# Genomics-HSE/MiSTI

Measured on AMD Instinct MI355X. Metric: composite-llk evals/sec over (split×mi) grid, 128 merged PSMC intervals, higher is better.
Workload: dtype f64; 1 GPU; config2: numT=128, 64x64 split x mi-rate grid, one band, --cpfit; candidates_per_gpu=4096, candidates_total=4096, replicates=1, numT=128, batches_in_flight=20, streams=20, world_size=1, parallelism=1 GPU

## Files before the change

misti_amd/csrc/misti_api.cpp:

```cpp
#include <cassert>
#include <hip/hip_runtime.h>

#include <cmath>
#include <chrono>
#include <complex>
#include <thread>
#include <cstdarg>
#include <cstdio>
#include <cstring>
#include <mutex>
#include <string>
#include <vector>

#include "misti_device.h"
#include "misti_tables.hpp"

namespace {

thread_local std::string g_err;

int fail(int code, const char* fmt, ...) {
    char buf[512];
    va_list ap;
    va_start(ap, fmt);
// ... 37 lines not shown
        size_t want = bytes + bytes / 4 + 4096;
        hipError_t e = hipHostMalloc(&p, want, hipHostMallocDefault);
        if (e == hipSuccess) cap = want;
        return e;
    }
    void release() { if (p) (void)hipHostFree(p); p = nullptr; cap = 0; }
};
constexpr size_t PIN_STAGE_MAX = (size_t)256 << 20;

}

struct misti_ctx {
    int device = 0;
    misti::DevModel dm{};
    int unfolded = 0;
    hipStream_t own_stream = nullptr;
    hipStream_t stream = nullptr;
    DevBuf model_f64, model_i32;
    DevBuf consts;
    DevBuf scan_v, scan_i;
    DevBuf prof_v, prof_i, prof_idx;
    DevBuf ws_jafs, ws_status;
    DevBuf ws_order;
    DevBuf ws_diag;
    int64_t diag_n = 0;
    int32_t* hint_host = nullptr;
    int32_t* hint_dev = nullptr;
    int32_t batch_seq = 0;
    misti::Tuning tune;
    int table_cur = 0;
    size_t table_clean[2] = {0, 0};
    DevBuf ws_trunk;
    DevBuf ws_chain_f64, ws_chain_i32;
    DevBuf st_split, st_params, st_bounds, st_pulses, st_jsfs, st_llk, st_jafs, st_lc, st_pr, st_status;
    PinBuf pin_in, pin_out;
    std::vector<char> heap_in, heap_out;
    bool trace = false;
    DevBuf ws_solver, ws_iters;
    DevBuf ws_post;
    int64_t trace_n = 0, trace_iter_cap = 0;
    const int32_t* trace_of = nullptr;
    hipEvent_t order_ev = nullptr;
    hipEvent_t last_ev = nullptr;
    bool last_ev_set = false;
    unsigned hints = 0;
    hipStream_t side_stream = nullptr;
// ... 149 lines not shown
    if (n_cand == 0) return 0;
    if (!d_split) return fail(MISTI_E_ARG, "split_time is NULL");
    if (c->hints & MISTI_HINT_INTEGER_SPLITS) hints |= RUN_INTEGER_SPLITS;
    if (c->dm.n_param > 0 && !d_params) return fail(MISTI_E_ARG, "params is NULL but the model has %d parameters", c->dm.n_param);
    if (n_rep > 0 && (!d_jsfs || !d_llk)) return fail(MISTI_E_ARG, "jsfs / llk is NULL with n_rep > 0");
    HIP_TRY(hipSetDevice(c->device));
    if (!d_jafs) { HIP_TRY(c->ws_jafs.reserve((size_t)n_cand * 7 * sizeof(double))); d_jafs = c->ws_jafs.as<double>(); }
    if (!d_status) { HIP_TRY(c->ws_status.reserve((size_t)n_cand * sizeof(int32_t))); d_status = c->ws_status.as<int32_t>(); }
    if (n_cand > INT32_MAX / 8) return fail(MISTI_E_LIMIT, "n_cand too large for one call");
    const size_t nc = (size_t)n_cand, numT = (size_t)c->dm.numT;
    const size_t tsize = misti::chain_table_size(n_cand);
    const int64_t follow_max_h = c->tune.follow_max > 0 ? c->tune.follow_max : misti::FOLLOW_MAX_CHAINS;
    const size_t ntr = ((hints & RUN_UNSHARED) && n_cand > follow_max_h) ? 0 : (size_t)misti::trunk_capacity(n_cand, c->tune);
    const size_t f64_n = nc * numT * 2 + nc * (numT + 1) * 6 + nc * 6 + nc * 2 + nc * 6;
    const size_t set_n = 4 + 4 * tsize;
    const size_t i32_n = 2 * set_n + 10 * nc + ntr;
    HIP_TRY(c->ws_chain_f64.reserve(f64_n * sizeof(double)));
    {
        void* before = c->ws_chain_i32.p;
        HIP_TRY(c->ws_chain_i32.reserve(i32_n * sizeof(int32_t)));
        if (c->ws_chain_i32.p != before) c->table_clean[0] = c->table_clean[1] = 0;
    }
    HIP_TRY(c->ws_order.reserve(nc * sizeof(int32_t)));
    if (ntr) HIP_TRY(c->ws_trunk.reserve(ntr * numT * misti::TRUNK_REC * sizeof(double)));
    if (n_rep > 0) HIP_TRY(c->consts.reserve((size_t)n_rep * sizeof(double)));
    misti::ChainBufs cb;
    {
        double* d = c->ws_chain_f64.as<double>();
        cb.lc = d; d += nc * numT * 2;
        cb.trace = d; d += nc * (numT + 1) * 6;
        cb.work = d; d += nc * 6;
        cb.tail_lc = d; d += nc * 2;
        cb.tail_state = d;
        int32_t* q = c->ws_chain_i32.as<int32_t>();
        const int cur = c->table_cur;
        int32_t* set[2] = {q, q + set_n};
        q += 2 * set_n;
        if (c->table_clean[cur] != tsize) HIP_TRY(hipMemsetAsync(set[cur], 0, set_n * sizeof(int32_t), c->stream));
        c->table_clean[cur] = 0;
        c->table_clean[cur ^ 1] = 0;
        cb.n_chains = set[cur]; cb.table = set[cur] + 4; cb.slot_chain = cb.table + tsize; cb.slot_len = cb.slot_chain + tsize;
        cb.slot_keep = cb.slot_len + tsize;
        cb.z_n_chains = set[cur ^ 1]; cb.z_table = set[cur ^ 1] + 4; cb.z_slot_len = cb.z_table + 2 * tsize; cb.z_slot_keep = cb.z_slot_len + tsize;
        cb.slot_of = q; q += nc; cb.of = q; q += nc; cb.chain_slot = q; q += nc; cb.rep = q; q += nc;
        cb.fail_t = q; q += nc; cb.fail_status = q; q += nc; cb.tail_status = q; q += nc; cb.chain_order = q; q += nc; cb.resume_t = q; q += nc; cb.resume_list = q; q += nc;
        cb.trunk_ok = q;
        cb.tmask = (uint32_t)(tsize - 1);
        cb.trunk = ntr ? c->ws_trunk.as<double>() : nullptr;
        cb.trunk_cap = (int64_t)ntr;
        cb.hint = c->hint_dev;
        cb.simd_load = c->tune.pairing ? pair_table(c->device) : nullptr;
        cb.bounds = c->dm.n_band > 0 ? d_bounds : nullptr;
        cb.pulse_times = c->dm.n_pulse > 0 ? d_pulses : nullptr;
        cb.integer_splits = (hints & RUN_INTEGER_SPLITS) ? 1 : 0;
        cb.post_lam = nullptr;
        cb.post_word = nullptr;
        if (!(c->dm.flags & MISTI_CPFIT)) {
            HIP_TRY(c->ws_post.reserve(nc * (numT + 1) * (sizeof(double) + sizeof(int32_t))));
            cb.post_lam = c->ws_post.as<double>();
            if (c->trace) cb.post_word = reinterpret_cast<int32_t*>(cb.post_lam + nc * (numT + 1));
        }
        cb.solver = cb.tail_solver = cb.cand_solver = nullptr;
        cb.iters = nullptr;
        cb.iter_cap = 0;
        c->trace_n = 0;
        c->trace_iter_cap = 0;
        if (c->trace) {
            HIP_TRY(c->ws_solver.reserve((nc * numT + nc + nc * (numT + 1)) * sizeof(int32_t)));
            HIP_TRY(hipMemsetAsync(c->ws_solver.p, 0, (nc * numT + nc + nc * (numT + 1)) * sizeof(int32_t), c->stream));
// ... 280 lines not shown
    if (hipEventCreateWithFlags(&c->last_ev, hipEventDisableTiming) != hipSuccess) { (void)hipGetLastError(); c->last_ev = nullptr; }
    {
        std::lock_guard<std::mutex> lock(g_ctx_mu);
        g_ctxs.push_back(c);
    }
    guard.keep = true;
    *out = c;
    return 0;
}

int misti_create(const misti_model_t* model, int device, misti_ctx** out) { return misti_create_prio_(model, device, 0, out); }

int misti_destroy(misti_ctx* c) {
    if (!c) return 0;
    {
        std::lock_guard<std::mutex> lock(g_ctx_mu);
        for (size_t i = 0; i < g_ctxs.size(); ++i) if (g_ctxs[i] == c) { g_ctxs.erase(g_ctxs.begin() + (long)i); break; }
    }
    (void)hipSetDevice(c->device);
    if (c->stream) (void)hipStreamSynchronize(c->stream);
    if (c->own_stream && c->own_stream != c->stream) (void)hipStreamSynchronize(c->own_stream);
    if (c->side_stream) (void)hipStreamSynchronize(c->side_stream);
    (void)hipGetLastError();
    for (auto* b : {&c->model_f64, &c->model_i32, &c->consts, &c->ws_jafs, &c->ws_status, &c->ws_chain_f64, &c->ws_chain_i32, &c->ws_order, &c->ws_diag, &c->ws_trunk, &c->ws_solver, &c->ws_iters, &c->ws_post,
                    &c->st_split, &c->st_params, &c->st_bounds, &c->st_pulses, &c->st_jsfs, &c->st_llk, &c->st_jafs, &c->st_lc, &c->st_pr, &c->st_status, &c->nm_f64, &c->nm_i32, &c->scan_v, &c->scan_i, &c->prof_v, &c->prof_i, &c->prof_idx, &c->curv_f64, &c->curv_i32, &c->boot_chunks, &c->param_totals})
        b->release();
    c->pin_in.release();
    c->pin_out.release();
    if (c->nm_live_host) (void)hipHostFree(c->nm_live_host);
    if (c->hint_host) (void)hipHostFree(c->hint_host);
    for (int w = 0; w < 3; ++w)
        for (auto& pr : c->pending[w]) { (void)hipEventDestroy(pr.first); (void)hipEventDestroy(pr.second); }
    for (hipEvent_t e : {c->order_ev, c->last_ev, c->packed_ev, c->side_ev}) if (e) (void)hipEventDestroy(e);
    if (c->side_stream) (void)hipStreamDestroy(c->side_stream);
    if (c->own_stream) (void)hipStreamDestroy(c->own_stream);
    (void)hipGetLastError();
    delete c;
    return 0;
}

int misti_set_stream(misti_ctx* c, void* s) {
    if (!c) return fail(MISTI_E_ARG, "ctx is NULL");
    hipStream_t next = s ? static_cast<hipStream_t>(s) : c->own_stream;
    if (next == c->stream) return 0;
    HIP_TRY(hipSetDevice(c->device));
    if (!c->order_ev) HIP_TRY(hipEventCreateWithFlags(&c->order_ev, hipEventDisableTiming));
    HIP_TRY(hipEventRecord(c->order_ev, c->stream));
// ... 1046 lines not shown
```

misti_amd/csrc/misti_device.h:

```cpp
#pragma once
#include <hip/hip_runtime.h>
#include <stdint.h>

#include "../../include/misti_hip.h"

#include "misti_consts.h"

namespace misti {

struct DevTables {
    int src[MAXNZ][64];
    int kind[MAXNZ][64];
    int mult[MAXNZ][64];
    int dcnt[4][64];
    int jaf[7][64];
    int jaf1[7][NS1];
    unsigned long long jaf_bits[7][3];
    unsigned int jaf1_bits[7];
    int grp_lo[NS1], grp_hi[NS1];
    int anc_n[2], anc_dst[2], anc_src[2][8];
    int pulse_n[2][64];
    int pulse_src[2][64][MAXPULSE];
    int pulse_ab[2][64][MAXPULSE];
    double tal_zr[TALBOT_HALF], tal_zi[TALBOT_HALF];
    double tal_cr[TALBOT_HALF], tal_ci[TALBOT_HALF];
};

struct DevModel {
    int numT;
    int sample_date;
    unsigned flags;
    int n_band, n_pulse, n_param;
    double mixture_th;
    const double* times;
    const double* lh;
    const int* run_start;
    const int* run_end;
    const int* leave_ok;
    misti_band_t bands[MISTI_MAX_BANDS];
    misti_pulse_t pulses[MISTI_MAX_PULSES];
};

struct ChainBufs {
    int32_t* n_chains;
    int32_t* z_n_chains;
    int32_t* z_table;
    int32_t* z_slot_len;
    int32_t* z_slot_keep;
    int32_t* table;
    int32_t* slot_chain;
    int32_t* slot_len;
    int32_t* slot_keep;
    int32_t* resume_t;
    int32_t* resume_list;
    int32_t* chain_order;
    int32_t* slot_of;
    int32_t* of;
    int32_t* chain_slot;
    int32_t* rep;
    uint32_t tmask;
    double* lc;
    double* trace;
    int32_t* fail_t;
    int32_t* fail_status;
    double* work;
    double* tail_lc;
    double* tail_state;
    int32_t* tail_status;
    double* trunk;
    int32_t* trunk_ok;
    int64_t trunk_cap;
    int32_t* simd_load;
    int32_t* hint;
    int32_t seq;
    int32_t unsorted;
    int32_t integer_splits;
    const int32_t* bounds;
    const int32_t* pulse_times;
    double* post_lam;
    int32_t* post_word;
    int32_t* solver;
    int32_t* tail_solver;
    int32_t* cand_solver;
    double* iters;
    int64_t iter_cap;
};

__host__ __device__ __forceinline__ int32_t solver_word(int nfev, int status, int kind) {
    return (int32_t)((nfev & 0xffff) | ((status & 15) << 16) | ((kind & 15) << 20));
}

__device__ __forceinline__ int64_t chain_of(const ChainBufs& cb, int64_t cand) { return cb.of[cand]; }
__device__ __forceinline__ int chain_len(const ChainBufs& cb, int64_t ch) { return cb.slot_len[cb.chain_slot[ch]]; }

enum { NM_NONE = 0, NM_REFLECT = 1, NM_EXPAND = 2, NM_CONTRACT = 3, NM_INSIDE = 4,
       NM_CUT = 5 };
struct NmBatch {
    double* pts;
    double* split;
    int32_t* row;
    int32_t* bnd;
    int32_t* put;
    double* par;
};
enum { NM_B_INIT, NM_B_REFLECT, NM_B_SECOND, NM_B_SHRINK, NM_B_SPEC, NM_BATCHES };
struct NmState {
    int64_t S;
    int N;
    int maxiter;
    int64_t maxfun;
    double xatol, fatol;
    double split;
    const double* split_of;
    const int32_t* row_of;
    const int32_t* bounds_of;
// ... 120 lines not shown
```

misti_amd/csrc/misti_kernels.hip:

```cpp
#include <hip/hip_runtime.h>
#include <math.h>
#include <stdint.h>
#include <stdlib.h>

#include "misti_device.h"
#include "misti_score.h"

namespace misti {

__constant__ DevTables c_tab;
__constant__ double c_inv[INV_TABLE];
constexpr int QMAX_TABLE = 320;
__constant__ double c_qmax[QMAX_TABLE];

constexpr double Q_SWITCH = 96.0;
constexpr int JACOBI_MAX = 600;
constexpr int JACOBI_WATCH = 32;
constexpr int JACOBI_FLOOR = 48;
constexpr double JACOBI_BLOWUP = 1e12;
constexpr int SUBSTEP_MAX = 256;
constexpr long long FOLLOW_SPIN_LIMIT = 1LL << 22;

__device__ __forceinline__ int lane_id() { return threadIdx.x & 63; }

// ... 1686 lines not shown
#endif
#ifdef MISTI_STAMP
            r[0] = (double)c_tree; r[1] = (double)(c_collect + c_update); r[2] = (double)c_next;
            r[3] = (double)c_adv; r[4] = (double)c_batch; r[5] = (double)c_book;
#endif
        } else {
            cb.tail_status[cand] = status;
        }
    }
}

#ifndef MISTI_DEFAULT_FIT_WAVES
#define MISTI_DEFAULT_FIT_WAVES 1
#endif
#ifndef MISTI_FOLLOW_WAVES
#define MISTI_FOLLOW_WAVES 2
#endif
template <bool CPFIT, int GROUP>
__global__ __launch_bounds__(64) __attribute__((amdgpu_waves_per_eu(CPFIT ? 2 : MISTI_DEFAULT_FIT_WAVES, CPFIT ? 2 : MISTI_DEFAULT_FIT_WAVES)))
void correct_kernel(DevModel m, int64_t n_items, ChainBufs cb, const double* __restrict__ split_time, const double* __restrict__ params, int yield_nfev) {
    extern __shared__ double lds[];
    {
        const int64_t i = (int64_t)blockIdx.x * 64 + threadIdx.x;
        if (i < n_items) cb.of[i] = cb.slot_chain[cb.slot_of[i]];
    }
    correct_body<CPFIT, GROUP, false>(m, n_items, cb, split_time, params, (int64_t)blockIdx.x, lds, nullptr, nullptr, nullptr, cb.chain_order,
                                      GROUP == 64 ? 0 : yield_nfev);
}

template <bool CPFIT>
__global__ __launch_bounds__(64) __attribute__((amdgpu_waves_per_eu(CPFIT ? MISTI_FOLLOW_WAVES : 1, CPFIT ? MISTI_FOLLOW_WAVES : 1)))
void correct_resume_kernel(DevModel m, int64_t n_items, ChainBufs cb, const double* __restrict__ split_time, const double* __restrict__ params) {
    extern __shared__ double lds[];
    __shared__ int next;
    const int n_res = cb.n_chains[3];
    if ((int)blockIdx.x >= n_res) return;
    __builtin_amdgcn_s_setprio(3);
    double* pre = lds + 3 * (size_t)m.numT;
    for (;;) {
        if (threadIdx.x == 0) next = atomicAdd(&cb.n_chains[2], 1);
        __syncthreads();
        const int pos = next;
        __syncthreads();
        if (pos >= n_res) break;
        const int64_t ch = cb.resume_list[pos];
        correct_body<CPFIT, 64, false, true>(m, n_items, cb, split_time, params, ch, lds, nullptr, nullptr, pre, nullptr, 0, cb.resume_t[ch]);
        __syncthreads();
// ... 146 lines not shown
            const double gr = T * zr * zz, gi = -T * zi * zz;
            accp += 2.0 * wr;
            acci += 2.0 * (wr * gr - wi * gi);
        }
        if (solved) {
            x = accp; wint = acci;
        } else {
            const int n_sub = (int)ceil(q / Q_SWITCH);
            if (n_sub > SUBSTEP_MAX) return MISTI_STIFF;
            const double2 r = series_substeps(R.srcl[0], R.srcl[1], R.srcl[2], R.srcl[3], cf[0], cf[1], cf[2], cf[3], xbuf, lane, n_sub, q, T, dT, x);
            x = r.x; wint = r.y;
        }
    }
    if (t < m.sample_date) w_pre += wint; else w_post += wint;
    return MISTI_OK;
}

__device__ __forceinline__ double run_mean(const double* lc, int k, int a, int b, const Grid& G) {
    double acc = 0.0, tt = 0.0;
    for (int j = a; j < b; ++j) { double Tj = G.T(j); acc += lc[2 * j + k] * Tj; tt += Tj; }
    return acc / tt;
}

__device__ __forceinline__ void smooth_rates(const DevModel& m, const Grid& G, double* lcb, int lane, int lo, int bound) {
    double sm[SMOOTH_REPS][2];
#pragma unroll
    for (int rep = 0; rep < SMOOTH_REPS; ++rep) {
        sm[rep][0] = sm[rep][1] = 0.0;
        if (rep * 64 >= bound || rep * 64 + 63 < lo) continue;
        int t = rep * 64 + lane;
        for (int k = 0; k < 2; ++k) {
            double v = 0.0;
            if (t >= lo && t < bound) {
                int a = m.run_start[k * m.numT + t];
                int b = m.run_end[k * m.numT + t];
                if (b > bound) b = bound;
                v = run_mean(lcb, k, a, b, G);
            }
            sm[rep][k] = v;
        }
    }
    lds_fence();
#pragma unroll
    for (int rep = 0; rep < SMOOTH_REPS; ++rep) {
        int t = rep * 64 + lane;
        if (t >= lo && t < bound) { lcb[2 * t] = sm[rep][0]; lcb[2 * t + 1] = sm[rep][1]; }
    }
    lds_fence();
}

__device__ __forceinline__ bool trunk_active(const ChainBufs& cb, int64_t n_cand) {
    const int64_t nch = cb.n_chains[0];
    return cb.trunk_cap > 0 && nch <= cb.trunk_cap && nch * TRUNK_MIN_SHARE <= n_cand;
}

__device__ __forceinline__
void trunk_body(const DevModel& m, int64_t n_cand, const double* __restrict__ params, const ChainBufs& cb, int64_t ch, double* lds, int phase = 0) {
    const int lane = lane_id();
    if (!trunk_active(cb, n_cand) || ch >= cb.n_chains[0]) return;
    if (wrong_phase(cb, ch, phase)) return;
    double* xbuf = lds;
    double* lcb = lds + 128;
    const int ft = cb.fail_t[ch];
    int Lt = chain_len(cb, ch);
    if (ft < Lt) Lt = ft;
    const double* par = params ? params + (int64_t)cb.rep[ch] * m.n_param : nullptr;
    Grid G;
    G.times = m.times; G.lh = m.lh; G.numT0 = m.numT; G.numT = m.numT; G.split = Lt; G.ins = -1; G.frac = 0.0;
    Model mod{&m, par, Lt, {0, 0, 0, 0}};
    mod.bb = cb.bounds ? cb.bounds + (int64_t)cb.rep[ch] * 2 * m.n_band : nullptr;
    mod.pt = cb.pulse_times ? cb.pulse_times + (int64_t)cb.rep[ch] * m.n_pulse : nullptr;
// ... 80 lines not shown
        const int cut = have >= need ? len : have;
        if (t >= cut) break;
        if (b0 > cut) b0 = cut;
        if (b1 > cut) b1 = cut;
        const double l0 = smooth ? run_mean(lc_sh, 0, a0, b0, G) : lc_sh[2 * t];
        const double l1 = smooth ? run_mean(lc_sh, 1, a1, b1, G) : lc_sh[2 * t + 1];
        if (lane == 0) { lcb[2 * t] = l0; lcb[2 * t + 1] = l1; }
        lds_fence();
        if (t == m.sample_date) ancient_project(xbuf, lane, x);
        if (twopop_interval(R, m, mod, G, lcb, xbuf, lane, t, x, w_pre, w_post) != MISTI_OK) break;
    }
    if (!stored) store(ok, xs, ws0, ws1);
    if (lane == 0) cb.trunk_ok[ch] = ok;
}

template <bool CPFIT>
__global__ __launch_bounds__(128) __attribute__((amdgpu_waves_per_eu(CPFIT ? MISTI_FOLLOW_WAVES : 1, CPFIT ? MISTI_FOLLOW_WAVES : 1)))
void correct_follow_kernel(DevModel m, int64_t n_items, ChainBufs cb, const double* __restrict__ split_time, const double* __restrict__ params) {
    extern __shared__ double lds[];
    double* tk = lds + 3 * (size_t)m.numT;
    double* lc_sh = tk + 128 + 2 * (size_t)(m.numT + 1);
    volatile int* flags = (volatile int*)(lc_sh + 2 * (size_t)m.numT);
    double* pre = lc_sh + 2 * (size_t)m.numT + 4;
    for (int64_t i = (int64_t)blockIdx.x * 128 + threadIdx.x; i < n_items; i += (int64_t)gridDim.x * 128) cb.of[i] = cb.slot_chain[cb.slot_of[i]];
    const int64_t n_live = cb.n_chains[0];
    if ((int64_t)blockIdx.x >= n_live) return;
    int* next = (int*)(flags + 2);
    bool chain_role = threadIdx.x < 64;
    int32_t* my_load = nullptr;
    if (cb.simd_load) {
        int* ex = next + 1;
        const unsigned hw = __builtin_amdgcn_s_getreg((31 << 11) | 4);
        const unsigned xcc = __builtin_amdgcn_s_getreg((3 << 11) | 20);
        const int simd = (hw >> 4) & 3;
        if ((threadIdx.x & 63) == 0) ex[threadIdx.x >> 6] = simd;
        if (threadIdx.x == 0) ex[2] = (int)((((xcc & 7) * 8 + ((hw >> 13) & 7)) * 2 + ((hw >> 12) & 1)) * 16 + ((hw >> 8) & 15)) * 4;
        __syncthreads();
        if (threadIdx.x == 0) {
            int32_t* t = cb.simd_load + ex[2];
            const int c0 = __hip_atomic_load(&t[ex[0]], __ATOMIC_RELAXED, __HIP_MEMORY_SCOPE_AGENT);
            const int c1 = __hip_atomic_load(&t[ex[1]], __ATOMIC_RELAXED, __HIP_MEMORY_SCOPE_AGENT);
            const int sw = c1 < c0 ? 1 : 0;
            ex[3] = sw;
            atomicAdd(&t[ex[sw]], 1);
        }
        __syncthreads();
        chain_role = ((int)(threadIdx.x >> 6) ^ ex[3]) == 0;
// ... 56 lines not shown
    const double lh0 = G.lhk(t, 0), lh1 = G.lhk(t, 1);
    const double pa = exp(nc0), pb = exp(nc1);
    const double w0 = pa / (pa + pb), w1 = pb / (pa + pb);
    const double Te = w0 * ect_one_pop(lh0, T) + w1 * ect_one_pop(lh1, T);
    double x[1] = {w0 * lh0 + w1 * lh1};
    auto resid = [&](const double l[1], double f[1]) { f[0] = ect_one_pop(l[0], T) - Te; };
    const int32_t word = trf_bounded<1>(resid, x, 0.01 * fmin(lh0, lh1));
    cb.post_lam[gid] = x[0];
    if (cb.post_word) cb.post_word[gid] = word;
}

template <bool CPFIT, int WPB = WAVES_PER_BLOCK>
__global__ __launch_bounds__(WPB * 64, 4)
void spectrum_kernel(DevModel m, int64_t n_cand, const int32_t* __restrict__ order, const double* __restrict__ split_time, const double* __restrict__ params,
                     ChainBufs cb, double* __restrict__ lc_out, double* __restrict__ pr_out,
                     double* __restrict__ jafs_out, int32_t* __restrict__ status_out, double* __restrict__ diag_out,
                     int n_inline, const double* __restrict__ jsfs, const double* __restrict__ consts, double* __restrict__ llk_out, int phase) {
    extern __shared__ double lds[];
    const int lane = lane_id();
    const int wave = __builtin_amdgcn_readfirstlane((int)(threadIdx.x >> 6));
    const int64_t slot = (int64_t)blockIdx.x * WPB + wave;
    if (slot >= n_cand) return;
    if (phase != 0) {
        const int64_t cd = (int64_t)__builtin_amdgcn_readfirstlane(order[slot]);
        if (wrong_phase(cb, (int64_t)__builtin_amdgcn_readfirstlane((int)chain_of(cb, cd)), phase)) return;
    }
#ifdef MISTI_STAMP2
    long long s_[8];
#define KSTAMP(i) s_[i] = clock64();
#else
#define KSTAMP(i)
#endif
    KSTAMP(0)
    const int64_t cand = (int64_t)__builtin_amdgcn_readfirstlane(order[slot]);
    const int lc_rows = m.numT + 1;
    double* xbuf = lds + (size_t)wave * (128 + 2 * lc_rows);
    double* lcb = xbuf + 128;
    const double* par = params ? params + cand * m.n_param : nullptr;
    Grid G;
    const int32_t* bb = cb.bounds ? cb.bounds + cand * 2 * m.n_band : nullptr;
    const int32_t* pt = cb.pulse_times ? cb.pulse_times + cand * m.n_pulse : nullptr;
    int status = setup_candidate(m, split_time[cand], par, G, bb, pt);
    if (status == MISTI_OK && cb.integer_splits && G.ins >= 0) status = MISTI_BAD_STRUCTURE;
    Model mod{&m, par, G.split, {0, 0, 0, 0}};
    mod.bb = bb;
    mod.pt = pt;
    mod.cache();
    const int64_t ch = (int64_t)__builtin_amdgcn_readfirstlane((int)chain_of(cb, cand));
    const int nfull = (G.ins >= 0) ? G.ins : G.split;
    const double* lc_ch = cb.lc + ch * (int64_t)m.numT * 2;
    const double* tr_ch = cb.trace + ch * (int64_t)(m.numT + 1) * 6;
    int have = 0;
    if (status == MISTI_OK) {
        const int ft = cb.fail_t[ch];
        if (ft < nfull) { status = cb.fail_status[ch]; have = ft + 1; }
        else {
            have = nfull;
            if (G.ins >= 0) { const int ts = cb.tail_status[cand]; have = nfull + 1; if (ts != MISTI_OK) status = ts; }
        }
    }
    double* lc_o = lc_out ? lc_out + cand * (int64_t)lc_rows * 2 : nullptr;
    double* pr_o = pr_out ? pr_out + cand * (int64_t)(m.numT + 2) * 6 : nullptr;
    int32_t* sv_o = cb.cand_solver ? cb.cand_solver + cand * (int64_t)lc_rows : nullptr;
    if (sv_o) {
        for (int i = lane; i < lc_rows; i += 64) {
            int32_t wd = 0;
            if (i < nfull && i < have) wd = cb.solver[ch * (int64_t)m.numT + i];
            else if (i == nfull && G.ins >= 0 && have > nfull) wd = cb.tail_solver[cand];
            sv_o[i] = wd;
        }
    }
    if (pr_o) {
        const int rows = (status == MISTI_OK) ? G.split + 1 : (have > nfull ? nfull + 1 : (have > 0 ? have : (status == MISTI_OK ? 1 : 0)));
        for (int i = lane; i < (m.numT + 2) * 6; i += 64) {
            const int r = i / 6, j = i - 6 * r;
            double v = 0.0;
            if (r == m.numT + 1) v = cb.work[ch * 6 + j];
            else if (r < rows) v = (G.ins >= 0 && r == nfull + 1) ? cb.tail_state[cand * 6 + j] : tr_ch[6 * r + j];
            pr_o[i] = v;
        }
    }
    if (status != MISTI_OK) {
        if (lane == 0) { status_out[cand] = status; if (diag_out) diag_out[cand] = NAN; }
        if (lane < 7) jafs_out[cand * 7 + lane] = NAN;
        if (lane < n_inline) llk_out[cand * n_inline + lane] = -INFINITY;
        if (lc_o)
            for (int i = lane; i < 2 * lc_rows; i += 64) {
                const int t = i >> 1;
                lc_o[i] = (t < have && t < nfull) ? lc_ch[i] : (t < have && t == nfull && G.ins >= 0) ? cb.tail_lc[2 * cand + (i & 1)] : 0.0;
            }
        return;
    }
    KSTAMP(1)
    for (int i = lane; i < 2 * lc_rows; i += 64) {
        const int t = i >> 1;
        lcb[i] = (t < nfull) ? lc_ch[i] : (t == nfull && G.ins >= 0) ? cb.tail_lc[2 * cand + (i & 1)] : 0.0;
    }
    lds_fence();
    {
        double mx = 0.0;
        for (int t = lane; t < G.split; t += 64) { double T = G.T(t); mx = fmax(mx, fmax(lcb[2 * t], lcb[2 * t + 1]) * T); }
        for (int o = 32; o > 0; o >>= 1) mx = fmax(mx, __shfl_xor(mx, o, 64));
        if (diag_out && lane == 0) diag_out[cand] = (m.flags & MISTI_TRUE_EPS) ? 0.0 : mx;
    }
    int t0 = 0;
    const bool use_trunk = trunk_active(cb, n_cand);
    int smooth_from = 0;
    if (use_trunk) {
        const int t_own = trunk_leave(m, G);
        t0 = min(t_own, cb.trunk_ok[ch]);
        if (t0 == t_own && !lc_o) smooth_from = t_own;
    }
    KSTAMP(2)
    {
        const double* stt = (G.ins >= 0) ? cb.tail_state + 6 * cand : tr_ch + 6 * nfull;
        const double nc0 = (stt[0] + stt[2]) + stt[4], nc1 = (stt[1] + stt[3]) + stt[5];
        const double delta = nc1 - nc0;
        const double ed = exp(delta);
        const int last = G.numT - 1;
        for (int base = G.split; base < G.numT; base += 64) {
            int t = base + lane;
            if (t < last) {
                double T = G.T(t);
                double lam = 1.0;
                int32_t word = 0;
                if (T != 0) {
                    double lh0 = G.lhk(t, 0), lh1 = G.lhk(t, 1);
                    if (CPFIT) {
                        double pnc = (exp(-T * lh0) + exp(delta - T * lh1)) / (1.0 + ed);
                        lam = -log(pnc) / T;
                        word = solver_word(0, 0, 1);
                    } else {
                        lam = cb.post_lam[cand * lc_rows + t];
                        word = cb.post_word ? cb.post_word[cand * lc_rows + t] : 0;
                    }
                }
                lcb[2 * t] = lam; lcb[2 * t + 1] = lam;
                if (sv_o) sv_o[t] = word;
            } else if (t == last) {
                double lh0 = G.lhk(t, 0), lh1 = G.lhk(t, 1);
                double lam = (1.0 + ed) / (1.0 / lh0 + ed / lh1);
                lcb[2 * t] = lam; lcb[2 * t + 1] = lam;
                if (sv_o) sv_o[t] = solver_word(0, 0, 1);
            }
        }
        lds_fence();
        KSTAMP(3)
        if (m.flags & MISTI_SMOOTH) smooth_rates(m, G, lcb, lane, smooth_from, G.split);
        for (int i = lane; i < 2 * G.numT; i += 64) { double v = lcb[i]; if (!(v == v)) status = MISTI_NUMERIC; }
        status = __any(status != MISTI_OK) ? MISTI_NUMERIC : MISTI_OK;
        if (lc_o) for (int i = lane; i < 2 * lc_rows; i += 64) lc_o[i] = (i < 2 * G.numT) ? lcb[i] : 0.0;
    }
    double jn = NAN;
    KSTAMP(4)
    KSTAMP(5) KSTAMP(6) KSTAMP(7)

    if (status == MISTI_OK) {
        TwoPopRow R;
        R.load(lane);
        const bool live = R.live;
        double x = (lane == 2) ? 1.0 : 0.0;
        double w_pre = 0.0, w_post = 0.0;
        if (use_trunk) {
            const double* r = cb.trunk + (ch * (int64_t)m.numT + t0) * TRUNK_REC;
            if (live) { x = r[lane]; w_pre = r[NS2 + lane]; w_post = r[2 * NS2 + lane]; }
        }
        for (int t = t0; t <= G.split && t < G.numT; ++t) {
            if (t == m.sample_date) ancient_project(xbuf, lane, x);
            if (t == G.split) break;
            const int st = twopop_interval(R, m, mod, G, lcb, xbuf, lane, t, x, w_pre, w_post);
            if (st != MISTI_OK) { status = st; break; }
        }
        KSTAMP(5)
        if (status == MISTI_OK) {
            double jp;
            {
                double a4[4], a2[2], z;
                {
                    double a[8];
#pragma unroll
                    for (int c = 0; c < 7; ++c) {
                        const double wg = (double)c_tab.jaf[c][lane];
                        a[c] = live ? (c < 2 ? wg * w_post + wg * w_pre : wg * w_post) : 0.0;
                    }
                    a[7] = 0.0;
                    const bool hi = lane & 32;
#pragma unroll
                    for (int c = 0; c < 4; ++c) { const double keep = hi ? a[c + 4] : a[c], give = hi ? a[c] : a[c + 4]; a4[c] = keep + __shfl_xor(give, 32, 64); }
                }
// ... 126 lines not shown
#pragma unroll
            for (int u = 0; u < SORT_ILP; ++u) if (i0 + u * (int64_t)blockDim.x < n) atomicAdd(&hist[key(st[u])], 1);
        }
        __syncthreads();
        __shared__ int bin_base[MISTI_MAX_NUMT + 4];
        for (int b = threadIdx.x; b < nb; b += blockDim.x) {
            int acc = 0;
            for (int c = 0; c < SORT_SUB; ++c) { const int v = hist[b * SORT_SUB + c]; hist[b * SORT_SUB + c] = acc; acc += v; }
            bin_base[b] = acc;
        }
        __syncthreads();
        if (threadIdx.x == 0) { int acc = 0; for (int b = 0; b < nb; ++b) { const int c = bin_base[b]; bin_base[b] = acc; acc += c; } }
        __syncthreads();
        for (int b = threadIdx.x; b < nb; b += blockDim.x) for (int c = 0; c < SORT_SUB; ++c) hist[b * SORT_SUB + c] += bin_base[b];
        __syncthreads();
        for (int64_t i0 = threadIdx.x; i0 < n; i0 += step) {
            double st[SORT_ILP];
            int pos[SORT_ILP];
#pragma unroll
            for (int u = 0; u < SORT_ILP; ++u) { const int64_t i = i0 + u * (int64_t)blockDim.x; st[u] = i < n ? split_time[i] : 0.0; }
#pragma unroll
            for (int u = 0; u < SORT_ILP; ++u) pos[u] = i0 + u * (int64_t)blockDim.x < n ? atomicAdd(&hist[key(st[u])], 1) : 0;
#pragma unroll
            for (int u = 0; u < SORT_ILP; ++u) { const int64_t i = i0 + u * (int64_t)blockDim.x; if (i < n) order[pos[u]] = (int32_t)i; }
        }
        return;
    }
    const int64_t i = (int64_t)blockIdx.x * blockDim.x + threadIdx.x;
    {
        const int64_t tsize = (int64_t)cb.tmask + 1, nthr = (int64_t)cand_blocks * blockDim.x;
        for (int64_t k = i; k < tsize; k += nthr) { cb.z_table[k] = 0; cb.z_slot_len[k] = 0; cb.z_slot_keep[k] = 0; }
        if (i == 0) { cb.z_n_chains[0] = 0; cb.z_n_chains[1] = 0; cb.z_n_chains[2] = 0; cb.z_n_chains[3] = 0; }
    }
    if (i < n) {
        if (cb.unsorted & 1) order[i] = (int32_t)i;
        uint64_t h = 0x243f6a8885a308d3ull;
        const double* a = params + i * P;
        const int32_t* ab = cb.bounds ? cb.bounds + i * NB2 : nullptr;
        for (int k = 0; k < P; ++k) h = mix64(h ^ (uint64_t)__double_as_longlong(a[k]));
        if (ab) for (int k = 0; k < NB2; ++k) h = mix64(h ^ (uint64_t)(uint32_t)ab[k]);
        const int32_t* ap = cb.pulse_times ? cb.pulse_times + i * NPU : nullptr;
        if (ap) for (int k = 0; k < NPU; ++k) h = mix64(h ^ (uint64_t)(uint32_t)ap[k]);
        const double st = split_time[i];
        if (!(st >= 0)) h = mix64(h ^ (uint64_t)i);
        uint32_t sl = (uint32_t)(h >> 20) & cb.tmask;
        for (;;) {
            const int prev = atomicCAS(&cb.table[sl], 0, (int)i + 1);
            if (prev == 0) {
                const int ch = atomicAdd(cb.n_chains, 1);
                cb.chain_slot[ch] = (int32_t)sl;
                cb.rep[ch] = (int32_t)i;
                cb.slot_chain[sl] = ch;
                if (cb.unsorted & 2) cb.chain_order[ch] = ch;
                break;
            }
            const double* b = params + (int64_t)(prev - 1) * P;
            bool same = true;
            for (int k = 0; k < P; ++k) if (__double_as_longlong(a[k]) != __double_as_longlong(b[k])) same = false;
            if (ab) { const int32_t* bbp = cb.bounds + (int64_t)(prev - 1) * NB2; for (int k = 0; k < NB2; ++k) if (ab[k] != bbp[k]) same = false; }
            if (ap) { const int32_t* pp = cb.pulse_times + (int64_t)(prev - 1) * NPU; for (int k = 0; k < NPU; ++k) if (ap[k] != pp[k]) same = false; }
            if (same) break;
            sl = (sl + 1) & cb.tmask;
        }
        cb.slot_of[i] = (int32_t)sl;
        int need = 0;
        if (st >= 0 && st <= (double)numT) { need = (int)st; if (need > numT - 1) need = numT - 1; }
        atomicMax(&cb.slot_len[sl], need);
        Grid G;
        if (setup_candidate(m, st, P ? a : nullptr, G, ab, ap) == MISTI_OK) {
            int t_own = trunk_leave(m, G);
            t_own = t_own < 0 ? 0 : (t_own > numT - 1 ? numT - 1 : t_own);
            atomicMax(&cb.slot_keep[sl], numT - t_own);
        }
    }
    __shared__ int is_last;
    __syncthreads();
    if (threadIdx.x == 0) {
        __threadfence();
        is_last = atomicAdd(&cb.n_chains[1], 1) == cand_blocks - 1;
    }
    __syncthreads();
    if (!is_last) return;
    __threadfence();
    const int nch = __hip_atomic_load(cb.n_chains, __ATOMIC_RELAXED, __HIP_MEMORY_SCOPE_AGENT);
    if (cb.unsorted & 2) {
        if (cb.hint && threadIdx.x == 0) { cb.hint[0] = nch; cb.hint[1] = (int32_t)n; __threadfence_system(); cb.hint[2] = cb.seq; }
        return;
    }
    auto len_of = [&](int ch) {
        const int sl = __hip_atomic_load(&cb.chain_slot[ch], __ATOMIC_RELAXED, __HIP_MEMORY_SCOPE_AGENT);
        const int L = __hip_atomic_load(&cb.slot_len[sl], __ATOMIC_RELAXED, __HIP_MEMORY_SCOPE_AGENT);
        return numT - (L < 0 ? 0 : (L > numT ? numT : L));
    };
    for (int k = threadIdx.x; k < numT + 2; k += blockDim.x) hist[k] = 0;
    __syncthreads();
    for (int ch = threadIdx.x; ch < nch; ch += blockDim.x) atomicAdd(&hist[len_of(ch)], 1);
// ... 31 lines not shown
    for (int k = 1; k < INV_TABLE; ++k) inv[k] = 1.0 / (double)k;
    hipError_t e = hipMemcpyToSymbol(HIP_SYMBOL(c_inv), inv, sizeof inv);
    if (e != hipSuccess) return e;
    {
        static double qmax[QMAX_TABLE];
        qmax[0] = -1.0; qmax[1] = -1.0;
        const long double tol = logl(1e-19L);
        for (int K = 2; K < QMAX_TABLE; ++K) {
            long double lo = 0.0L, hi = (long double)(K - 1);
            for (int it = 0; it < 200; ++it) {
                const long double mid = 0.5L * (lo + hi);
                const long double lw = -mid + (long double)(K - 1) * logl(mid) - lgammal((long double)K);
                if (lw < tol) lo = mid; else hi = mid;
            }
            qmax[K] = (double)lo;
        }
        qmax[QMAX_TABLE - 1] = 1e300;
        e = hipMemcpyToSymbol(HIP_SYMBOL(c_qmax), qmax, sizeof qmax);
        if (e != hipSuccess) return e;
    }
    return hipMemcpyToSymbol(HIP_SYMBOL(c_tab), &t, sizeof(DevTables));
}

size_t spectrum_lds_bytes(int numT, int wpb) { return (size_t)wpb * (128 + 2 * (numT + 1)) * sizeof(double); }

int correct_cands_per_wave(int64_t n_items, const Tuning& tn) {
    const int forced = tn.cands_per_wave;
    if (forced == 1 || forced == 2 || forced == 4 || forced == 8 || forced == 10) return forced;
    int cpw = 1;
    while (cpw < 8 && n_items / cpw > 2048) cpw *= 2;
    return cpw == 8 ? 10 : cpw;
}

Tuning read_tuning() {
    Tuning t;
    auto num = [](const char* name) { const char* e = getenv(name); return e ? atoi(e) : 0; };
    auto flag = [](const char* name) { const char* e = getenv(name); return e && e[0] && e[0] != '0'; };
    t.chains_per_wave = num("MISTI_CHAINS_PER_WAVE");
    t.cands_per_wave = num("MISTI_CANDS_PER_WAVE");
    t.no_follow = flag("MISTI_NO_FOLLOW");
    t.no_trunk = flag("MISTI_NO_TRUNK");
    t.follow_max = num("MISTI_FOLLOW_MAX_CHAINS");
    t.min_blocks = num("MISTI_FOLLOW_MIN_BLOCKS");
    t.busy_contexts = getenv("MISTI_FOLLOW_BUSY_CONTEXTS") ? num("MISTI_FOLLOW_BUSY_CONTEXTS") : -1;
    t.yield_nfev = getenv("MISTI_YIELD_NFEV") ? num("MISTI_YIELD_NFEV") : -1;
    t.k2_single_waves = getenv("MISTI_K2_SINGLE_WAVES") ? num("MISTI_K2_SINGLE_WAVES") : -1;
    t.pairing = !(getenv("MISTI_FOLLOW_PAIRING") && getenv("MISTI_FOLLOW_PAIRING")[0] == '0');
// ... 123 lines not shown
```

Before: 23.20 million llk evals/s.

## Precompute per-candidate setup records in sorted order for spectrum kernel

The hashing/sort pass now stores each candidate's setup results (split, insertion index, fraction, status, trunk-leave time) in a 32-byte record, and the resolve step scatters these records, with the chain id filled in, into the sorted order. The spectrum kernel then reads one contiguous record per slot instead of redoing setup_candidate, chasing order and chain indirections, and recomputing trunk_leave. The NaN check moves into the places where values are written, the lc load is fused with the diag max, and trunk and row loads are hoisted. Times are also staged into LDS per wave. This costs extra workspace, LDS and global writes, and relies on the Grid fields being fully rebuilt from the record.

New measurement: 23.33 million llk evals/s, median of 6. No clear change (+0.6%).

```diff
diff --git a/misti_amd/csrc/misti_api.cpp b/misti_amd/csrc/misti_api.cpp
--- a/misti_amd/csrc/misti_api.cpp
+++ b/misti_amd/csrc/misti_api.cpp
@@ -83,6 +83,7 @@
     DevBuf prof_v, prof_i, prof_idx;
     DevBuf ws_jafs, ws_status;
     DevBuf ws_order;
+    DevBuf ws_rec;
     DevBuf ws_diag;
     int64_t diag_n = 0;
     int32_t* hint_host = nullptr;
@@ -278,6 +279,7 @@
         if (c->ws_chain_i32.p != before) c->table_clean[0] = c->table_clean[1] = 0;
     }
     HIP_TRY(c->ws_order.reserve(nc * sizeof(int32_t)));
+    HIP_TRY(c->ws_rec.reserve(2 * nc * sizeof(misti::CandRec) + nc * sizeof(int32_t)));
     if (ntr) HIP_TRY(c->ws_trunk.reserve(ntr * numT * misti::TRUNK_REC * sizeof(double)));
     if (n_rep > 0) HIP_TRY(c->consts.reserve((size_t)n_rep * sizeof(double)));
     misti::ChainBufs cb;
@@ -301,6 +303,9 @@
         cb.slot_of = q; q += nc; cb.of = q; q += nc; cb.chain_slot = q; q += nc; cb.rep = q; q += nc;
         cb.fail_t = q; q += nc; cb.fail_status = q; q += nc; cb.tail_status = q; q += nc; cb.chain_order = q; q += nc; cb.resume_t = q; q += nc; cb.resume_list = q; q += nc;
         cb.trunk_ok = q;
+        cb.rec = c->ws_rec.as<misti::CandRec>();
+        cb.rec_in = cb.rec + nc;
+        cb.slot_pos = reinterpret_cast<int32_t*>(cb.rec_in + nc);
         cb.tmask = (uint32_t)(tsize - 1);
         cb.trunk = ntr ? c->ws_trunk.as<double>() : nullptr;
         cb.trunk_cap = (int64_t)ntr;
@@ -627,7 +632,7 @@
     if (c->own_stream && c->own_stream != c->stream) (void)hipStreamSynchronize(c->own_stream);
     if (c->side_stream) (void)hipStreamSynchronize(c->side_stream);
     (void)hipGetLastError();
-    for (auto* b : {&c->model_f64, &c->model_i32, &c->consts, &c->ws_jafs, &c->ws_status, &c->ws_chain_f64, &c->ws_chain_i32, &c->ws_order, &c->ws_diag, &c->ws_trunk, &c->ws_solver, &c->ws_iters, &c->ws_post,
+    for (auto* b : {&c->model_f64, &c->model_i32, &c->consts, &c->ws_jafs, &c->ws_status, &c->ws_chain_f64, &c->ws_chain_i32, &c->ws_order, &c->ws_rec, &c->ws_diag, &c->ws_trunk, &c->ws_solver, &c->ws_iters, &c->ws_post,
                     &c->st_split, &c->st_params, &c->st_bounds, &c->st_pulses, &c->st_jsfs, &c->st_llk, &c->st_jafs, &c->st_lc, &c->st_pr, &c->st_status, &c->nm_f64, &c->nm_i32, &c->scan_v, &c->scan_i, &c->prof_v, &c->prof_i, &c->prof_idx, &c->curv_f64, &c->curv_i32, &c->boot_chunks, &c->param_totals})
         b->release();
     c->pin_in.release();
diff --git a/misti_amd/csrc/misti_device.h b/misti_amd/csrc/misti_device.h
--- a/misti_amd/csrc/misti_device.h
+++ b/misti_amd/csrc/misti_device.h
@@ -1,5 +1,6 @@
 #pragma once
 #include <hip/hip_runtime.h>
+#include <stddef.h>
 #include <stdint.h>
 
 #include "../../include/misti_hip.h"
@@ -40,6 +41,17 @@
     misti_band_t bands[MISTI_MAX_BANDS];
     misti_pulse_t pulses[MISTI_MAX_PULSES];
 };
+
+struct alignas(32) CandRec {
+    int32_t cand;
+    int32_t chain;
+    int32_t status;
+    int32_t split;
+    int32_t ins;
+    int32_t t_own;
+    double frac;
+};
+static_assert(sizeof(CandRec) == 32 && offsetof(CandRec, chain) == 4, "resolve_candidate copies a CandRec as two int4");
 
 struct ChainBufs {
     int32_t* n_chains;
@@ -84,6 +96,9 @@
     int32_t* cand_solver;
     double* iters;
     int64_t iter_cap;
+    int32_t* slot_pos;
+    CandRec* rec_in;
+    CandRec* rec;
 };
 
 __host__ __device__ __forceinline__ int32_t solver_word(int nfev, int status, int kind) {
@@ -91,6 +106,17 @@
 }
 
 __device__ __forceinline__ int64_t chain_of(const ChainBufs& cb, int64_t cand) { return cb.of[cand]; }
+__device__ __forceinline__ void resolve_candidate(const ChainBufs& cb, int64_t i) {
+    const int32_t ch = cb.slot_chain[cb.slot_of[i]];
+    const int4* src = reinterpret_cast<const int4*>(cb.rec_in + i);
+    int4* dst = reinterpret_cast<int4*>(cb.rec + cb.slot_pos[i]);
+    int4 lo = src[0];
+    const int4 hi = src[1];
+    cb.of[i] = ch;
+    lo.y = ch;
+    dst[0] = lo;
+    dst[1] = hi;
+}
 __device__ __forceinline__ int chain_len(const ChainBufs& cb, int64_t ch) { return cb.slot_len[cb.chain_slot[ch]]; }
 
 enum { NM_NONE = 0, NM_REFLECT = 1, NM_EXPAND = 2, NM_CONTRACT = 3, NM_INSIDE = 4,
diff --git a/misti_amd/csrc/misti_kernels.hip b/misti_amd/csrc/misti_kernels.hip
--- a/misti_amd/csrc/misti_kernels.hip
+++ b/misti_amd/csrc/misti_kernels.hip
@@ -1732,7 +1732,7 @@
     extern __shared__ double lds[];
     {
         const int64_t i = (int64_t)blockIdx.x * 64 + threadIdx.x;
-        if (i < n_items) cb.of[i] = cb.slot_chain[cb.slot_of[i]];
+        if (i < n_items) resolve_candidate(cb, i);
     }
     correct_body<CPFIT, GROUP, false>(m, n_items, cb, split_time, params, (int64_t)blockIdx.x, lds, nullptr, nullptr, nullptr, cb.chain_order,
                                       GROUP == 64 ? 0 : yield_nfev);
@@ -1925,7 +1925,8 @@
     return acc / tt;
 }
 
-__device__ __forceinline__ void smooth_rates(const DevModel& m, const Grid& G, double* lcb, int lane, int lo, int bound) {
+template <bool CHECK = false>
+__device__ __forceinline__ bool smooth_rates(const DevModel& m, const Grid& G, double* lcb, int lane, int lo, int bound) {
     double sm[SMOOTH_REPS][2];
 #pragma unroll
     for (int rep = 0; rep < SMOOTH_REPS; ++rep) {
@@ -1944,12 +1945,14 @@
         }
     }
     lds_fence();
+    bool bad = false;
 #pragma unroll
     for (int rep = 0; rep < SMOOTH_REPS; ++rep) {
         int t = rep * 64 + lane;
-        if (t >= lo && t < bound) { lcb[2 * t] = sm[rep][0]; lcb[2 * t + 1] = sm[rep][1]; }
+        if (t >= lo && t < bound) { lcb[2 * t] = sm[rep][0]; lcb[2 * t + 1] = sm[rep][1]; if (CHECK) bad |= !(sm[rep][0] == sm[rep][0]) || !(sm[rep][1] == sm[rep][1]); }
     }
     lds_fence();
+    return bad;
 }
 
 __device__ __forceinline__ bool trunk_active(const ChainBufs& cb, int64_t n_cand) {
@@ -2076,7 +2079,7 @@
     double* lc_sh = tk + 128 + 2 * (size_t)(m.numT + 1);
     volatile int* flags = (volatile int*)(lc_sh + 2 * (size_t)m.numT);
     double* pre = lc_sh + 2 * (size_t)m.numT + 4;
-    for (int64_t i = (int64_t)blockIdx.x * 128 + threadIdx.x; i < n_items; i += (int64_t)gridDim.x * 128) cb.of[i] = cb.slot_chain[cb.slot_of[i]];
+    for (int64_t i = (int64_t)blockIdx.x * 128 + threadIdx.x; i < n_items; i += (int64_t)gridDim.x * 128) resolve_candidate(cb, i);
     const int64_t n_live = cb.n_chains[0];
     if ((int64_t)blockIdx.x >= n_live) return;
     int* next = (int*)(flags + 2);
@@ -2179,8 +2182,7 @@
     const int64_t slot = (int64_t)blockIdx.x * WPB + wave;
     if (slot >= n_cand) return;
     if (phase != 0) {
-        const int64_t cd = (int64_t)__builtin_amdgcn_readfirstlane(order[slot]);
-        if (wrong_phase(cb, (int64_t)__builtin_amdgcn_readfirstlane((int)chain_of(cb, cd)), phase)) return;
+        if (wrong_phase(cb, (int64_t)__builtin_amdgcn_readfirstlane(cb.rec[slot].chain), phase)) return;
     }
 #ifdef MISTI_STAMP2
     long long s_[8];
@@ -2189,31 +2191,44 @@
 #define KSTAMP(i)
 #endif
     KSTAMP(0)
-    const int64_t cand = (int64_t)__builtin_amdgcn_readfirstlane(order[slot]);
+    const CandRec* rp = cb.rec + slot;
+    const int64_t cand = (int64_t)__builtin_amdgcn_readfirstlane(rp->cand);
+    const int64_t ch = (int64_t)__builtin_amdgcn_readfirstlane(rp->chain);
+    int status = __builtin_amdgcn_readfirstlane(rp->status);
     const int lc_rows = m.numT + 1;
-    double* xbuf = lds + (size_t)wave * (128 + 2 * lc_rows);
+    double* xbuf = lds + (size_t)wave * (128 + 2 * lc_rows + m.numT);
     double* lcb = xbuf + 128;
+    double* tms = lcb + 2 * lc_rows;
+    for (int i = lane; i < m.numT - 1; i += 64) tms[i] = m.times[i];
     const double* par = params ? params + cand * m.n_param : nullptr;
     Grid G;
+    G.times = m.times; G.lh = m.lh; G.numT0 = m.numT;
+    G.frac = bcast(rp->frac, 0);
+    G.split = __builtin_amdgcn_readfirstlane(rp->split);
+    G.ins = __builtin_amdgcn_readfirstlane(rp->ins);
+    G.numT = G.ins >= 0 ? m.numT + 1 : m.numT;
     const int32_t* bb = cb.bounds ? cb.bounds + cand * 2 * m.n_band : nullptr;
     const int32_t* pt = cb.pulse_times ? cb.pulse_times + cand * m.n_pulse : nullptr;
-    int status = setup_candidate(m, split_time[cand], par, G, bb, pt);
     if (status == MISTI_OK && cb.integer_splits && G.ins >= 0) status = MISTI_BAD_STRUCTURE;
     Model mod{&m, par, G.split, {0, 0, 0, 0}};
     mod.bb = bb;
     mod.pt = pt;
     mod.cache();
-    const int64_t ch = (int64_t)__builtin_amdgcn_readfirstlane((int)chain_of(cb, cand));
     const int nfull = (G.ins >= 0) ? G.ins : G.split;
     const double* lc_ch = cb.lc + ch * (int64_t)m.numT * 2;
     const double* tr_ch = cb.trace + ch * (int64_t)(m.numT + 1) * 6;
     int have = 0;
+    bool use_trunk = false;
+    int trunk_ok = 0;
     if (status == MISTI_OK) {
-        const int ft = cb.fail_t[ch];
-        if (ft < nfull) { status = cb.fail_status[ch]; have = ft + 1; }
+        const int ft = cb.fail_t[ch], fs = cb.fail_status[ch];
+        const int ts = (G.ins >= 0) ? cb.tail_status[cand] : MISTI_OK;
+        use_trunk = trunk_active(cb, n_cand);
+        if (use_trunk) trunk_ok = cb.trunk_ok[ch];
+        if (ft < nfull) { status = fs; have = ft + 1; }
         else {
             have = nfull;
-            if (G.ins >= 0) { const int ts = cb.tail_status[cand]; have = nfull + 1; if (ts != MISTI_OK) status = ts; }
+            if (G.ins >= 0) { have = nfull + 1; if (ts != MISTI_OK) status = ts; }
         }
     }
     double* lc_o = lc_out ? lc_out + cand * (int64_t)lc_rows * 2 : nullptr;
@@ -2249,24 +2264,36 @@
         return;
     }
     KSTAMP(1)
-    for (int i = lane; i < 2 * lc_rows; i += 64) {
-        const int t = i >> 1;
-        lcb[i] = (t < nfull) ? lc_ch[i] : (t == nfull && G.ins >= 0) ? cb.tail_lc[2 * cand + (i & 1)] : 0.0;
-    }
-    lds_fence();
+    int t0 = 0;
+    int smooth_from = 0;
+    if (use_trunk) {
+        const int t_own = __builtin_amdgcn_readfirstlane(rp->t_own);
+        t0 = min(t_own, trunk_ok);
+        if (t0 == t_own && !lc_o) smooth_from = t_own;
+    }
+    TwoPopRow R;
+    R.load(lane);
+    const bool live = R.live;
+    double x = (lane == 2) ? 1.0 : 0.0;
+    double w_pre = 0.0, w_post = 0.0;
+    if (use_trunk) {
+        const double* r = cb.trunk + (ch * (int64_t)m.numT + t0) * TRUNK_REC;
+        if (live) { x = r[lane]; w_pre = r[NS2 + lane]; w_post = r[2 * NS2 + lane]; }
+    }
+    bool bad = false;
     {
         double mx = 0.0;
-        for (int t = lane; t < G.split; t += 64) { double T = G.T(t); mx = fmax(mx, fmax(lcb[2 * t], lcb[2 * t + 1]) * T); }
-        for (int o = 32; o > 0; o >>= 1) mx = fmax(mx, __shfl_xor(mx, o, 64));
-        if (diag_out && lane == 0) diag_out[cand] = (m.flags & MISTI_TRUE_EPS) ? 0.0 : mx;
-    }
-    int t0 = 0;
-    const bool use_trunk = trunk_active(cb, n_cand);
-    int smooth_from = 0;
-    if (use_trunk) {
-        const int t_own = trunk_leave(m, G);
-        t0 = min(t_own, cb.trunk_ok[ch]);
-        if (t0 == t_own && !lc_o) smooth_from = t_own;
+        for (int t = lane; t < G.split; t += 64) {
+            const double* src = (t < nfull) ? lc_ch + 2 * t : cb.tail_lc + 2 * cand;
+            const double v0 = src[0], v1 = src[1];
+            lcb[2 * t] = v0; lcb[2 * t + 1] = v1;
+            bad |= !(v0 == v0) || !(v1 == v1);
+            if (diag_out) mx = fmax(mx, fmax(v0, v1) * G.T(t));
+        }
+        if (diag_out) {
+            for (int o = 32; o > 0; o >>= 1) mx = fmax(mx, __shfl_xor(mx, o, 64));
+            if (lane == 0) diag_out[cand] = (m.flags & MISTI_TRUE_EPS) ? 0.0 : mx;
+        }
     }
     KSTAMP(2)
     {
@@ -2293,19 +2320,21 @@
                     }
                 }
                 lcb[2 * t] = lam; lcb[2 * t + 1] = lam;
+                bad |= !(lam == lam);
                 if (sv_o) sv_o[t] = word;
             } else if (t == last) {
                 double lh0 = G.lhk(t, 0), lh1 = G.lhk(t, 1);
                 double lam = (1.0 + ed) / (1.0 / lh0 + ed / lh1);
                 lcb[2 * t] = lam; lcb[2 * t + 1] = lam;
+                bad |= !(lam == lam);
                 if (sv_o) sv_o[t] = solver_word(0, 0, 1);
             }
         }
+        G.times = tms;
         lds_fence();
         KSTAMP(3)
-        if (m.flags & MISTI_SMOOTH) smooth_rates(m, G, lcb, lane, smooth_from, G.split);
-        for (int i = lane; i < 2 * G.numT; i += 64) { double v = lcb[i]; if (!(v == v)) status = MISTI_NUMERIC; }
-        status = __any(status != MISTI_OK) ? MISTI_NUMERIC : MISTI_OK;
+        if (m.flags & MISTI_SMOOTH) bad |= smooth_rates<true>(m, G, lcb, lane, smooth_from, G.split);
+        status = __any(bad) ? MISTI_NUMERIC : MISTI_OK;
         if (lc_o) for (int i = lane; i < 2 * lc_rows; i += 64) lc_o[i] = (i < 2 * G.numT) ? lcb[i] : 0.0;
     }
     double jn = NAN;
@@ -2313,15 +2342,6 @@
     KSTAMP(5) KSTAMP(6) KSTAMP(7)
 
     if (status == MISTI_OK) {
-        TwoPopRow R;
-        R.load(lane);
-        const bool live = R.live;
-        double x = (lane == 2) ? 1.0 : 0.0;
-        double w_pre = 0.0, w_post = 0.0;
-        if (use_trunk) {
-            const double* r = cb.trunk + (ch * (int64_t)m.numT + t0) * TRUNK_REC;
-            if (live) { x = r[lane]; w_pre = r[NS2 + lane]; w_post = r[2 * NS2 + lane]; }
-        }
         for (int t = t0; t <= G.split && t < G.numT; ++t) {
             if (t == m.sample_date) ancient_project(xbuf, lane, x);
             if (t == G.split) break;
@@ -2494,7 +2514,7 @@
 #pragma unroll
             for (int u = 0; u < SORT_ILP; ++u) pos[u] = i0 + u * (int64_t)blockDim.x < n ? atomicAdd(&hist[key(st[u])], 1) : 0;
 #pragma unroll
-            for (int u = 0; u < SORT_ILP; ++u) { const int64_t i = i0 + u * (int64_t)blockDim.x; if (i < n) order[pos[u]] = (int32_t)i; }
+            for (int u = 0; u < SORT_ILP; ++u) { const int64_t i = i0 + u * (int64_t)blockDim.x; if (i < n) { order[pos[u]] = (int32_t)i; cb.slot_pos[i] = pos[u]; } }
         }
         return;
     }
@@ -2505,7 +2525,7 @@
         if (i == 0) { cb.z_n_chains[0] = 0; cb.z_n_chains[1] = 0; cb.z_n_chains[2] = 0; cb.z_n_chains[3] = 0; }
     }
     if (i < n) {
-        if (cb.unsorted & 1) order[i] = (int32_t)i;
+        if (cb.unsorted & 1) { order[i] = (int32_t)i; cb.slot_pos[i] = (int32_t)i; }
         uint64_t h = 0x243f6a8885a308d3ull;
         const double* a = params + i * P;
         const int32_t* ab = cb.bounds ? cb.bounds + i * NB2 : nullptr;
@@ -2539,11 +2559,17 @@
         if (st >= 0 && st <= (double)numT) { need = (int)st; if (need > numT - 1) need = numT - 1; }
         atomicMax(&cb.slot_len[sl], need);
         Grid G;
-        if (setup_candidate(m, st, P ? a : nullptr, G, ab, ap) == MISTI_OK) {
+        CandRec rc;
+        rc.cand = (int32_t)i; rc.chain = -1; rc.t_own = 0;
+        rc.status = setup_candidate(m, st, P ? a : nullptr, G, ab, ap);
+        rc.split = G.split; rc.ins = G.ins; rc.frac = G.frac;
+        if (rc.status == MISTI_OK) {
             int t_own = trunk_leave(m, G);
+            rc.t_own = t_own;
             t_own = t_own < 0 ? 0 : (t_own > numT - 1 ? numT - 1 : t_own);
             atomicMax(&cb.slot_keep[sl], numT - t_own);
         }
+        cb.rec_in[i] = rc;
     }
     __shared__ int is_last;
     __syncthreads();
@@ -2621,7 +2647,7 @@
     return hipMemcpyToSymbol(HIP_SYMBOL(c_tab), &t, sizeof(DevTables));
 }
 
-size_t spectrum_lds_bytes(int numT, int wpb) { return (size_t)wpb * (128 + 2 * (numT + 1)) * sizeof(double); }
+size_t spectrum_lds_bytes(int numT, int wpb) { return (size_t)wpb * (128 + 2 * (numT + 1) + numT) * sizeof(double); }
 
 int correct_cands_per_wave(int64_t n_items, const Tuning& tn) {
     const int forced = tn.cands_per_wave;
```
